# cg-tuwien/ppsurf

Hardware: AMD Instinct MI355X
Metric: occupancy query-points/sec @ res=257, 50NN (higher is better)
Workload: dtype f16x3

## Files before the change

include/ppsurf_amd_ext.h:

```cpp
#ifndef PPSURF_AMD_EXT_H
#define PPSURF_AMD_EXT_H
#include <stddef.h>
#include <stdint.h>

#ifdef __cplusplus
extern "C" {
#endif

int ppsx_blend_rgba_u8(const int64_t* idx, const float* d2, int64_t m, int k, const uint8_t* rgba, int64_t n, double eps, uint8_t* out,
                       void* stream);

int ppsx_trim_cell_slots(const float* pts, int64_t n, const float* lo, const float* hi, float h, float inv_h, uint64_t* table, int64_t capacity,
                         int64_t* slot, void* stream);
int ppsx_trim_face_support(const float* verts, int64_t nv, const int64_t* faces, int64_t nf, const float* pts, int64_t n, const float* lo,
                           const float* hi, float h, float inv_h, const uint64_t* table, int64_t capacity, const int64_t* order,
                           const int64_t* offsets, double r, uint8_t* support, void* stream);

int ppsx_smooth_half_edges(const int64_t* faces, int64_t nf, int64_t nv, int64_t* keys, void* stream);
int ppsx_smooth_pass(const double* x, int64_t nv, const int64_t* offsets, const int32_t* nbr, const int32_t* mult, int64_t ne, double s,
                     double* out, void* stream);

#ifdef __cplusplus
}
#endif
#endif
```

ppsurf_amd/build.py:

```python
import concurrent.futures
import os
import subprocess
import sys

HERE = os.path.dirname(os.path.abspath(__file__))
CSRC = os.path.join(HERE, 'csrc')
LIB = os.path.join(HERE, 'libppsurf_amd.so')
SOURCES = ['pps_decode.hip', 'pps_knn.hip', 'pps_grow.hip', 'pps_mc.hip', 'pps_mesh.hip', 'pps_fkaconv.hip', 'pps_sample.hip', 'pps_train.hip', 'pps_csr.hip', 'pps_fka_train.hip', 'pps_bn_train.hip',
           'pps_attn_train.hip', 'pps_rows_train.hip', 'pps_gemm_train.hip', 'pps_optim.hip', 'pps_eval.hip', 'pps_vis.hip', 'pps_scan.hip', 'pps_cloud.hip', 'pps_simplify.hip', 'pps_transfer.hip', 'pps_trim.hip', 'pps_smooth.hip', 'pps_pack.cpp']
HEADERS = ['pps_common.h', 'pps_fka_common.h', 'pps_rows_train_impl.h', 'pps_head_chain_impl.h', 'pps_sweep.h', 'pps_rng.h', 'pps_cells.h', 'pps_tri.h', os.path.join('..', '..', 'include', 'ppsurf_amd.h'),
           os.path.join('..', '..', 'include', 'ppsurf_amd_ext.h')]
FLAGS = ['--offload-arch=gfx950', '-O3', '-std=c++17', '-ffp-contract=off', '-fPIC']


def _newer(path, deps):
    if not os.path.isfile(path):
        return True
    t = os.path.getmtime(path)
    return any(os.path.getmtime(d) > t for d in deps if os.path.isfile(d))


def build(force=False, verbose=False, variant=None, defines=()):
    hipcc = os.environ.get('HIPCC', '/opt/rocm/bin/hipcc')
    lib = LIB if not variant else os.path.join(HERE, 'libppsurf_amd_{}.so'.format(variant))
    objdir = os.path.join(CSRC, 'build' + ('_' + variant if variant else ''))
    os.makedirs(objdir, exist_ok=True)
    headers = [os.path.join(CSRC, h) for h in HEADERS]
    srcs = [s for s in SOURCES if os.path.isfile(os.path.join(CSRC, s))]
    jobs = []
    for s in srcs:
        src, obj = os.path.join(CSRC, s), os.path.join(objdir, os.path.splitext(s)[0] + '.o')
        if force or _newer(obj, [src] + headers):
            jobs.append([hipcc] + FLAGS + list(defines) + ['-c', src, '-o', obj])
    if jobs:
        def run(cmd):
            if verbose:
                print(' '.join(cmd), flush=True)
            return subprocess.run(cmd, stdout=subprocess.PIPE, stderr=subprocess.STDOUT, text=True)
        with concurrent.futures.ThreadPoolExecutor(max_workers=min(8, len(jobs))) as pool:
            for res in pool.map(run, jobs):
                if res.returncode != 0:
                    sys.stderr.write(res.stdout)
                    raise subprocess.CalledProcessError(res.returncode, res.args)
                if verbose and res.stdout.strip():
                    print(res.stdout)
    objs = [os.path.join(objdir, os.path.splitext(s)[0] + '.o') for s in srcs]
    if jobs or _newer(lib, objs):
        subprocess.check_call([hipcc, '--offload-arch=gfx950', '-shared', '-fPIC'] + objs + ['-o', lib])
    return lib


if __name__ == '__main__':
    argv = sys.argv[1:]
    variant, defines = None, [a for a in argv if a.startswith(('-D', '-f', '-m'))]
    if '--variant' in argv:
        variant = argv[argv.index('--variant') + 1]
    print(build(force='--force' in argv, verbose=True, variant=variant, defines=defines))
```

ppsurf_amd/csrc/pps_decode.hip:

```cpp
#include <cstdlib>
#include "pps_common.h"
#include "../../include/ppsurf_amd.h"

using namespace pps;

#ifndef NT
#define NT 256
#endif
#define NW (NT / 64)
#ifndef WG_PER_CU
#define WG_PER_CU (512 / NT)
#endif
#ifndef PPS_PRIO
#define PPS_PRIO 1
#endif
#ifndef PPS_PRIO_PN
#define PPS_PRIO_PN 1
#endif
#define CH4 2048

template <int CHUNK_F4_NEXT, int NTH = NT, class F>
__device__ __forceinline__ void stream_step(const f32x4* __restrict__ gnext, f32x4*& cur, f32x4*& nxt, F&& compute) {
    chunk_copy_async<CHUNK_F4_NEXT / NTH, NTH>(gnext, nxt);
    compute((const f32x4*)cur);
    stream_wait();
    __syncthreads();
    f32x4* t = cur; cur = nxt; nxt = t;
}

template <int CHUNK_F4_NEXT, int NTH = NT, class F>
__device__ __forceinline__ void stream_step_spread(const f32x4* __restrict__ gnext, f32x4*& cur, f32x4*& nxt, F&& compute) {
    f32x4* dst = nxt;
    compute((const f32x4*)cur, [&](int i) { if (i < CHUNK_F4_NEXT / NTH) chunk_copy_piece<NTH>(gnext, dst, i); });
    stream_wait();
    __syncthreads();
    f32x4* t = cur; cur = nxt; nxt = t;
}

template <int CHUNK_F4_NEXT, int NTH = NT, class F>
__device__ __forceinline__ void stream_step_spread_at(const char* chunk, const unsigned (&voff)[CHUNK_F4_NEXT / NTH], f32x4*& cur, f32x4*& nxt, F&& compute) {
    f32x4* dst = nxt;
    compute((const f32x4*)cur, [&](int i) { if (i < CHUNK_F4_NEXT / NTH) chunk_copy_piece_at<NTH>(chunk, dst, i, voff[i]); });
    stream_wait();
    __syncthreads();
    f32x4* t = cur; cur = nxt; nxt = t;
}

template <int CHUNK_F4, int NTH = NT>
__device__ __forceinline__ void stream_prologue(const f32x4* __restrict__ g, f32x4* buf) {
    chunk_copy_async<CHUNK_F4 / NTH, NTH>(g, buf);
}

__device__ __forceinline__ void lds_fill(float* dst, const float* __restrict__ src, int nfloats) {
    for (int i = threadIdx.x; i < nfloats; i += blockDim.x) dst[i] = src[i];
}
// ... 1195 lines not shown
    if (q < 0) return PPS_ERR_ARG;
    if (q == 0) return PPS_OK;
    if (!g || !wpack || !bias || !trans2) return PPS_ERR_ARG;
    static int once = set_lds(pointnet_stn_fc_kernel, PB_LDS_BYTES);
    (void)once;
    hipLaunchKernelGGL(pointnet_stn_fc_kernel, dim3(grid_for((q + NW * 16 * PB_T - 1) / (NW * 16 * PB_T))), dim3(NT), PB_LDS_BYTES, (hipStream_t)stream,
                       g, q, wpack, bias, trans2, gate);
    return PPS_LAUNCH_CHECK();
}

static int decode_tail_f32_impl(const float* pooled, const float* xbar, int64_t q, const float* wpack, const float* bias,
                                float* logits, float* occ, int* gate, void* stream) {
    if (q < 0) return PPS_ERR_ARG;
    if (q == 0) return PPS_OK;
    if (!pooled || !xbar || !wpack || !bias || !logits) return PPS_ERR_ARG;
    static int once = set_lds(decode_tail_kernel, TL_LDS_BYTES);
    (void)once;
    hipLaunchKernelGGL(decode_tail_kernel, dim3(grid_for((q + NW * 16 - 1) / (NW * 16))), dim3(NT), TL_LDS_BYTES, (hipStream_t)stream,
                       pooled, xbar, q, wpack, bias, logits, occ, gate);
    return PPS_LAUNCH_CHECK();
}

extern "C" {

int pps_abi_version(void) { return 2; }

int pps_debug_occupancy(int which) {
    int n = -1;
    if (which == 0) { set_lds(interp_pool_kernel, IP_LDS_BYTES); hipOccupancyMaxActiveBlocksPerMultiprocessor(&n, interp_pool_kernel, NT, IP_LDS_BYTES); }
    if (which == 1) { set_lds(pointnet_stn_rows_kernel<false>, PA_LDS_BYTES); hipOccupancyMaxActiveBlocksPerMultiprocessor(&n, pointnet_stn_rows_kernel<false>, PNT, PA_LDS_BYTES); }
    if (which == 3) { set_lds(pointnet_stn_fc_kernel, PB_LDS_BYTES); hipOccupancyMaxActiveBlocksPerMultiprocessor(&n, pointnet_stn_fc_kernel, NT, PB_LDS_BYTES); }
    if (which == 4) { set_lds(pointnet_stn_fc_h_kernel, PB_LDS_BYTES); hipOccupancyMaxActiveBlocksPerMultiprocessor(&n, pointnet_stn_fc_h_kernel, NT, PB_LDS_BYTES); }
    if (which == 2) { set_lds(pointnet_feat_rows_kernel<false>, PC_LDS_BYTES); hipOccupancyMaxActiveBlocksPerMultiprocessor(&n, pointnet_feat_rows_kernel<false>, PNT, PC_LDS_BYTES); }
    return n;
}
int pps_device_cu_count(void) { return cu_count(); }

int pps_rows_dense256_f32(const float* in, int64_t rs, int64_t cs, int64_t m, const float* wpack, const float* bias,
                          float* out, void* stream) {
    if (m < 0) return PPS_ERR_ARG;
    if (m == 0) return PPS_OK;
    if (!in || !wpack || !bias || !out) return PPS_ERR_ARG;
    if (cs == 1 && (rs % 4) != 0) return PPS_ERR_ARG;
    static int once = set_lds(rows_dense256_kernel, RD_LDS_BYTES);
    (void)once;
    hipLaunchKernelGGL(rows_dense256_kernel, dim3(grid_for((m + NW * 16 - 1) / (NW * 16))), dim3(NT), RD_LDS_BYTES, (hipStream_t)stream,
                       in, rs, cs, m, wpack, bias, out);
    return PPS_LAUNCH_CHECK();
}

int pps_interp_pool_f32(const float* G, const float* pts, const float* query, const int64_t* idx, int64_t q, int k,
                        const float* wpack, const float* bias, float* pooled, void* stream) {
    return interp_pool_f32_impl(G, pts, query, idx, q, k, wpack, bias, pooled, nullptr, stream);
}

int pps_interp_pool_f16x3(const float* G, const float* pts, const float* query, const int64_t* idx, int64_t q, int k,
                          const float* wxyz, const void* w16, const float* bias, float* pooled, int32_t* range_flag, void* stream) {
    if (q < 0 || k < 1 || k > 64) return PPS_ERR_ARG;
    if (q == 0) return PPS_OK;
    if (!G || !pts || !query || !idx || !wxyz || !w16 || !bias || !pooled) return PPS_ERR_ARG;
    static int once = set_lds(interp_pool_f16x3_kernel, IH_LDS_BYTES);
    (void)once;
    int cus = cu_count();
    if (cus <= 0) cus = 256;
    const int64_t ntiles = (q + IH_NW / 4 - 1) / (IH_NW / 4);
    const int64_t wgs = (int64_t)cus * IH_WG_PER_CU;
    const int grid = (int)(ntiles < wgs ? ntiles : wgs);
    hipLaunchKernelGGL(interp_pool_f16x3_kernel, dim3(grid), dim3(IH_NT), IH_LDS_BYTES, (hipStream_t)stream,
                       G, pts, query, idx, q, k, wxyz, (const f32x4*)w16, bias, pooled, (int*)range_flag);
    return PPS_LAUNCH_CHECK();
}

int pps_interp_small_f32(const float* G, const float* pts, const float* query, const int64_t* idx, int64_t q, int k, int c,
                         const float* wpack, const float* bias, const float* wtail, int nout, float* out, void* stream) {
    if (q < 0 || k < 1 || k > 64 || (c != 32 && c != 64) || nout < 1 || nout > IS_MAX_OUT) return PPS_ERR_ARG;
    if (q == 0) return PPS_OK;
    if (!G || !pts || !query || !idx || !wpack || !bias || !wtail || !out) return PPS_ERR_ARG;
    int cus = cu_count();
    if (cus <= 0) cus = 256;
    const int grid = (int)(q < (int64_t)cus * 8 ? q : (int64_t)cus * 8);
    hipStream_t st = (hipStream_t)stream;
    if (c == 32) hipLaunchKernelGGL((interp_small_kernel<2, false>), dim3(grid), dim3(IS_NT), 0, st, G, pts, query, idx, q, k, wpack, nullptr, bias, wtail, nout, out, nullptr);
    else hipLaunchKernelGGL((interp_small_kernel<4, false>), dim3(grid), dim3(IS_NT), 0, st, G, pts, query, idx, q, k, wpack, nullptr, bias, wtail, nout, out, nullptr);
    return PPS_LAUNCH_CHECK();
}

int pps_interp_small_f16x3(const float* G, const float* pts, const float* query, const int64_t* idx, int64_t q, int k, int c,
                           const float* wpack, const void* w16, const float* bias, const float* wtail, int nout, float* out, int* guard,
                           void* stream) {
    if (q < 0 || k < 1 || k > 64 || (c != 32 && c != 64) || nout < 1 || nout > IS_MAX_OUT) return PPS_ERR_ARG;
    if (q == 0) return PPS_OK;
    if (!G || !pts || !query || !idx || !wpack || !w16 || !bias || !wtail || !out || !guard) return PPS_ERR_ARG;
    int cus = cu_count();
    if (cus <= 0) cus = 256;
    const int grid = (int)(q < (int64_t)cus * 8 ? q : (int64_t)cus * 8);
    hipStream_t st = (hipStream_t)stream;
    if (hipMemsetAsync(guard, 0, sizeof(int), st) != hipSuccess) return PPS_ERR_LAUNCH;
    const float* wh = (const float*)w16;
    if (c == 32) {
        hipLaunchKernelGGL((interp_small_kernel<2, true>), dim3(grid), dim3(IS_NT), 0, st, G, pts, query, idx, q, k, wpack, wh, bias, wtail, nout, out, guard);
        hipLaunchKernelGGL((interp_small_kernel<2, false>), dim3(grid), dim3(IS_NT), 0, st, G, pts, query, idx, q, k, wpack, nullptr, bias, wtail, nout, out, guard);
    } else {
        hipLaunchKernelGGL((interp_small_kernel<4, true>), dim3(grid), dim3(IS_NT), 0, st, G, pts, query, idx, q, k, wpack, wh, bias, wtail, nout, out, guard);
        hipLaunchKernelGGL((interp_small_kernel<4, false>), dim3(grid), dim3(IS_NT), 0, st, G, pts, query, idx, q, k, wpack, nullptr, bias, wtail, nout, out, guard);
    }
    return PPS_LAUNCH_CHECK();
// ... 145 lines not shown
```

ppsurf_amd/csrc/pps_knn.hip:

```cpp
#include "pps_common.h"
#include "../../include/ppsurf_amd.h"

#define KNN_QW 8
#define KNN_WAVES 4
#define KNN_CAP 128
#ifndef KNN_BISECT
#define KNN_BISECT 12
#endif
#ifndef KNN_SEED
#define KNN_SEED 4
#endif

typedef unsigned long long u64;

__device__ __forceinline__ u64 shfl_xor_u64(u64 v, int m) {
    const int lo = __shfl_xor((int)(unsigned)v, m), hi = __shfl_xor((int)(unsigned)(v >> 32), m);
    return ((u64)(unsigned)hi << 32) | (unsigned)lo;
}
__device__ __forceinline__ u64 shfl_u64(u64 v, int src) {
    const int lo = __shfl((int)(unsigned)v, src), hi = __shfl((int)(unsigned)(v >> 32), src);
    return ((u64)(unsigned)hi << 32) | (unsigned)lo;
}

__device__ __forceinline__ float wave_min_f32(float v, int lane) {
    v = fminf(v, pps::dpp_mov<0xB1>(v));
    v = fminf(v, pps::dpp_mov<0x4E>(v));
    v = fminf(v, pps::dpp_mov<0x141>(v));
    v = fminf(v, pps::dpp_mov<0x140>(v));
    v = fminf(v, __uint_as_float(pps::lane_xor_u32(__float_as_uint(v), 16, lane)));
    v = fminf(v, __uint_as_float(pps::lane_xor_u32(__float_as_uint(v), 32, lane)));
    return v;
}

__device__ __forceinline__ u64 wave_sort64(u64 key, int lane) {
#pragma unroll
    for (int size = 2; size <= 64; size <<= 1) {
#pragma unroll
        for (int st = size >> 1; st > 0; st >>= 1) {
            const u64 other = pps::lane_xor_u64(key, st, lane);
            const bool up = ((lane & size) == 0);
            const bool lower = ((lane & st) == 0);
            const bool take_min = (up == lower);
            const u64 mn = key < other ? key : other, mx = key < other ? other : key;
            key = take_min ? mn : mx;
        }
    }
    return key;
}
__device__ __forceinline__ u64 wave_bitonic_merge64(u64 key, int lane) {
#pragma unroll
    for (int st = 32; st > 0; st >>= 1) {
        const u64 other = pps::lane_xor_u64(key, st, lane);
        const bool lower = ((lane & st) == 0);
        const u64 mn = key < other ? key : other, mx = key < other ? other : key;
        key = lower ? mn : mx;
    }
    return key;
}

__device__ __forceinline__ u64 knn_flush(u64 list, const u64* cand, int cnt, int lane) {
    while (cnt > 0) {
        const int c = cnt < 64 ? cnt : 64;
        u64 ck = (lane < c) ? cand[cnt - c + lane] : ~0ull;
// ... 31 lines not shown
            const int p = base + lane;
            const bool pv = p < n;
            const int pc = pv ? p : n - 1;
            const float px = pts[3 * pc], py = pts[3 * pc + 1], pz = pts[3 * pc + 2];
#pragma unroll
            for (int j = 0; j < KNN_QW; ++j) {
                const float dx = __fsub_rn(qx[j], px), dy = __fsub_rn(qy[j], py), dz = __fsub_rn(qz[j], pz);
                const float d2 = __fadd_rn(__fadd_rn(__fmul_rn(dx, dx), __fmul_rn(dy, dy)), __fmul_rn(dz, dz));
                const bool pass = pv && (d2 < tau[j]);
                const u64 mask = __ballot(pass);
                if (mask != 0ull) {
                    u64* cand = cand_all[wave][j];
                    const int pos = cnt[j] + (int)__builtin_amdgcn_mbcnt_hi((unsigned)(mask >> 32), __builtin_amdgcn_mbcnt_lo((unsigned)mask, 0));
                    if (pass) cand[pos] = ((u64)__float_as_uint(d2) << 32) | (unsigned)p;
                    cnt[j] += __popcll(mask);
                    if (cnt[j] > KNN_CAP - 64) {
                        list[j] = knn_flush(list[j], cand + (cnt[j] - 64), 64, lane);
                        cnt[j] -= 64;
                        tau[j] = __uint_as_float((unsigned)(shfl_u64(list[j], k - 1) >> 32));
                    }
                }
            }
        }
#pragma unroll
        for (int j = 0; j < KNN_QW; ++j) {
            list[j] = knn_flush(list[j], cand_all[wave][j], cnt[j], lane);
            if (q0 + j < m && lane < k) {
                out_idx[(q0 + j) * k + lane] = (int64_t)(unsigned)(list[j] & 0xffffffffull);
                if (out_d2) out_d2[(q0 + j) * k + lane] = __uint_as_float((unsigned)(list[j] >> 32));
            }
        }
    }
}

__device__ __forceinline__ void wave_merge2(u64& a, u64& b, int lane) {
    const u64 rev = shfl_u64(b, 63 - lane);
    const u64 lo = a < rev ? a : rev, hi = a < rev ? rev : a;
    a = wave_bitonic_merge64(lo, lane);
    b = wave_bitonic_merge64(hi, lane);
}

template <int R>
__device__ __forceinline__ void knn_flush_r(u64 (&list)[R], const u64* cand, int cnt, int lane) {
    while (cnt > 0) {
        const int c = cnt < 64 ? cnt : 64;
        u64 carry = (lane < c) ? cand[cnt - c + lane] : ~0ull;
        carry = wave_sort64(carry, lane);
#pragma unroll
        for (int r = 0; r < R; ++r) wave_merge2(list[r], carry, lane);
        cnt -= c;
    }
}

template <int R>
__global__ __launch_bounds__(KNN_WAVES * 64) void knn_blocked_kernel(const float* __restrict__ pts, const int* __restrict__ orig,
                                                                     const float* __restrict__ bbox, int nb,
                                                                     const float* __restrict__ win_bbox, int n_win,
                                                                     const float* __restrict__ sbox ,
                                                                     const float* __restrict__ query, int64_t m, int k,
                                                                     int64_t* __restrict__ out_idx, float* __restrict__ out_d2) {
    __shared__ u64 cand_all[KNN_WAVES][KNN_QW][KNN_CAP];
    const int ngrp = (nb + 63) >> 6;
    const int lane = threadIdx.x & 63, wave = threadIdx.x >> 6;
    const int kr = (k - 1) >> 6, kl = (k - 1) & 63;
    const int64_t ntask = (m + KNN_QW - 1) / KNN_QW;
    for (int64_t task = (int64_t)blockIdx.x * KNN_WAVES + wave; task < ntask; task += (int64_t)gridDim.x * KNN_WAVES) {
        const int64_t q0 = task * KNN_QW;
        float qx[KNN_QW], qy[KNN_QW], qz[KNN_QW], tau[KNN_QW];
        u64 list[KNN_QW][R];
        int cnt[KNN_QW], wbest[KNN_QW];
#pragma unroll
        for (int j = 0; j < KNN_QW; ++j) {
            const int64_t qq = (q0 + j < m) ? q0 + j : m - 1;
            qx[j] = __shfl(query[qq * 3], 0); qy[j] = __shfl(query[qq * 3 + 1], 0); qz[j] = __shfl(query[qq * 3 + 2], 0);
            tau[j] = INFINITY;
            wbest[j] = 0;
#pragma unroll
            for (int r = 0; r < R; ++r) list[j][r] = ~0ull;
            cnt[j] = 0;
        }
        if (sbox != nullptr && n_win > 0) {
#pragma unroll
            for (int j = 0; j < KNN_QW; ++j) {
                float best = INFINITY;
                int bw = 0;
                for (int g0 = 0; g0 * 64 < n_win; g0 += 64) {
                    const int g = g0 + lane;
                    const bool gv = g * 64 < n_win;
                    const float* gb = sbox + (int64_t)(gv ? g : 0) * 6;
                    const float gx = fmaxf(fmaxf(__fsub_rn(gb[0], qx[j]), __fsub_rn(qx[j], gb[3])), 0.f);
                    const float gy = fmaxf(fmaxf(__fsub_rn(gb[1], qy[j]), __fsub_rn(qy[j], gb[4])), 0.f);
                    const float gz = fmaxf(fmaxf(__fsub_rn(gb[2], qz[j]), __fsub_rn(qz[j], gb[5])), 0.f);
                    const float gnear = gv ? __fadd_rn(__fadd_rn(__fmul_rn(gx, gx), __fmul_rn(gy, gy)), __fmul_rn(gz, gz)) : INFINITY;
                    u64 pend = __ballot(gnear < best);
                    while (pend != 0ull) {
                        const bool mine = (pend >> lane) & 1ull;
                        const float tn = wave_min_f32(mine ? gnear : INFINITY, lane);
                        const int src = __builtin_ctzll(__ballot(mine && gnear == tn));
                        const int b = (g0 + src) * 64 + lane;
                        const bool bv = b < n_win;
                        const float* bb = win_bbox + (int64_t)(bv ? b : 0) * 6;
                        const float fx = fmaxf(fabsf(__fsub_rn(qx[j], bb[0])), fabsf(__fsub_rn(qx[j], bb[3])));
                        const float fy = fmaxf(fabsf(__fsub_rn(qy[j], bb[1])), fabsf(__fsub_rn(qy[j], bb[4])));
                        const float fz = fmaxf(fabsf(__fsub_rn(qz[j], bb[2])), fabsf(__fsub_rn(qz[j], bb[5])));
                        const float far2 = bv ? __fadd_rn(__fadd_rn(__fmul_rn(fx, fx), __fmul_rn(fy, fy)), __fmul_rn(fz, fz)) : INFINITY;
                        const float tf = wave_min_f32(far2, lane);
                        if (tf < best) {
                            best = tf;
                            bw = (g0 + src) * 64 + __builtin_ctzll(__ballot(far2 == tf));
                        }
                        pend &= ~(1ull << src);
                        pend &= __ballot(gnear < best);
                    }
                }
                tau[j] = best;
                wbest[j] = bw;
            }
        } else {
            for (int b0 = 0; b0 < n_win; b0 += 64) {
                const int b = b0 + lane;
                const bool bv = b < n_win;
                const float* bb = win_bbox + (int64_t)(bv ? b : 0) * 6;
                const float lx = bb[0], ly = bb[1], lz = bb[2], hx = bb[3], hy = bb[4], hz = bb[5];
#pragma unroll
                for (int j = 0; j < KNN_QW; ++j) {
                    const float fx = fmaxf(fabsf(__fsub_rn(qx[j], lx)), fabsf(__fsub_rn(qx[j], hx)));
                    const float fy = fmaxf(fabsf(__fsub_rn(qy[j], ly)), fabsf(__fsub_rn(qy[j], hy)));
                    const float fz = fmaxf(fabsf(__fsub_rn(qz[j], lz)), fabsf(__fsub_rn(qz[j], hz)));
                    const float far2 = bv ? __fadd_rn(__fadd_rn(__fmul_rn(fx, fx), __fmul_rn(fy, fy)), __fmul_rn(fz, fz)) : INFINITY;
                    if (far2 < tau[j]) { tau[j] = far2; wbest[j] = b; }
                }
            }
        }
        const int nfull = n_win > 0 ? n_win + R - 1 : 0;
        constexpr int SEEDS = KNN_SEED > R ? KNN_SEED : R;
        const int nseed = nfull < SEEDS ? nfull : SEEDS;
#pragma unroll
        for (int j = 0; j < KNN_QW; ++j) {
            const float t = wave_min_f32(tau[j], lane);
            const u64 who = __ballot(tau[j] == t);
            tau[j] = t;
            if (nseed > 0) {
                const int w = __shfl(wbest[j], who != 0ull ? __builtin_ctzll(who) : 0);
                int s0 = w - (nseed - R) / 2;
                s0 = s0 < 0 ? 0 : s0;
                s0 = s0 + nseed > nfull ? nfull - nseed : s0;
                unsigned u[SEEDS];
#pragma unroll
                for (int rr = 0; rr < SEEDS; ++rr) {
                    const int p = (s0 + (rr < nseed ? rr : 0)) * 64 + lane;
                    const float dx = __fsub_rn(qx[j], pts[3 * p]), dy = __fsub_rn(qy[j], pts[3 * p + 1]), dz = __fsub_rn(qz[j], pts[3 * p + 2]);
                    const float d2 = __fadd_rn(__fadd_rn(__fmul_rn(dx, dx), __fmul_rn(dy, dy)), __fmul_rn(dz, dz));
                    u[rr] = rr < nseed ? __float_as_uint(d2) : 0xffffffffu;
                }
                unsigned lo = 0u, hi = __float_as_uint(tau[j]);
                {
                    int c = 0;
#pragma unroll
                    for (int rr = 0; rr < SEEDS; ++rr) c += __popcll(__ballot(u[rr] <= hi));
                    if (c < k) lo = hi;
                }
#pragma unroll
                for (int it = 0; it < KNN_BISECT; ++it) {
                    const unsigned mid = lo + ((hi - lo) >> 1);
                    int c = 0;
#pragma unroll
                    for (int rr = 0; rr < SEEDS; ++rr) c += __popcll(__ballot(u[rr] <= mid));
                    if (c >= k) hi = mid; else lo = mid + (lo < hi ? 1u : 0u);
                }
                tau[j] = __uint_as_float(hi);
            }
        }
        for (int g0 = 0; g0 < ngrp; g0 += 64) {
          u64 gneed[KNN_QW];
          u64 gany = 0ull;
          {
            const int g = g0 + lane;
            const bool gv = g < ngrp;
            if (sbox != nullptr) {
                const float* bb = sbox + (int64_t)(gv ? g : 0) * 6;
                const float lx = bb[0], ly = bb[1], lz = bb[2], hx = bb[3], hy = bb[4], hz = bb[5];
#pragma unroll
                for (int j = 0; j < KNN_QW; ++j) {
                    const float gx = fmaxf(fmaxf(__fsub_rn(lx, qx[j]), __fsub_rn(qx[j], hx)), 0.f);
                    const float gy = fmaxf(fmaxf(__fsub_rn(ly, qy[j]), __fsub_rn(qy[j], hy)), 0.f);
                    const float gz = fmaxf(fmaxf(__fsub_rn(lz, qz[j]), __fsub_rn(qz[j], hz)), 0.f);
                    const float near2 = __fadd_rn(__fadd_rn(__fmul_rn(gx, gx), __fmul_rn(gy, gy)), __fmul_rn(gz, gz));
                    gneed[j] = __ballot(gv && near2 <= tau[j]);
                    gany |= gneed[j];
                }
            } else {
                gany = __ballot(gv);
#pragma unroll
                for (int j = 0; j < KNN_QW; ++j) gneed[j] = gany;
            }
          }
          while (gany != 0ull) {
            const int gbit = __builtin_ctzll(gany);
            gany &= gany - 1ull;
            const int b0 = (g0 + gbit) * 64;
            const int b = b0 + lane;
            const bool bv = b < nb;
            const float* bb = bbox + (int64_t)(bv ? b : 0) * 6;
            const float lx = bb[0], ly = bb[1], lz = bb[2], hx = bb[3], hy = bb[4], hz = bb[5];
            u64 need[KNN_QW];
            u64 any = 0ull;
#pragma unroll
            for (int j = 0; j < KNN_QW; ++j) {
                need[j] = 0ull;
                if (((gneed[j] >> gbit) & 1ull) == 0ull) continue;
                const float gx = fmaxf(fmaxf(__fsub_rn(lx, qx[j]), __fsub_rn(qx[j], hx)), 0.f);
                const float gy = fmaxf(fmaxf(__fsub_rn(ly, qy[j]), __fsub_rn(qy[j], hy)), 0.f);
                const float gz = fmaxf(fmaxf(__fsub_rn(lz, qz[j]), __fsub_rn(qz[j], hz)), 0.f);
                const float near2 = __fadd_rn(__fadd_rn(__fmul_rn(gx, gx), __fmul_rn(gy, gy)), __fmul_rn(gz, gz));
                need[j] = __ballot(bv && near2 <= tau[j]);
                any |= need[j];
            }
            while (any != 0ull) {
                const int bit = __builtin_ctzll(any);
                any &= any - 1ull;
                const int p = (b0 + bit) * 64 + lane;
                const float px = pts[3 * p], py = pts[3 * p + 1], pz = pts[3 * p + 2];
                const int oi = orig[p];
                const bool pv = oi >= 0;
#pragma unroll
                for (int j = 0; j < KNN_QW; ++j) {
                    if (((need[j] >> bit) & 1ull) == 0ull) continue;
                    const float dx = __fsub_rn(qx[j], px), dy = __fsub_rn(qy[j], py), dz = __fsub_rn(qz[j], pz);
                    const float d2 = __fadd_rn(__fadd_rn(__fmul_rn(dx, dx), __fmul_rn(dy, dy)), __fmul_rn(dz, dz));
                    const bool pass = pv && (d2 <= tau[j]);
                    const u64 mask = __ballot(pass);
                    if (mask != 0ull) {
                        u64* cand = cand_all[wave][j];
                        const int pos = cnt[j] + (int)__builtin_amdgcn_mbcnt_hi((unsigned)(mask >> 32), __builtin_amdgcn_mbcnt_lo((unsigned)mask, 0));
                        if (pass) cand[pos] = ((u64)__float_as_uint(d2) << 32) | (unsigned)oi;
                        cnt[j] += __popcll(mask);
                        if (cnt[j] > KNN_CAP - 64) {
                            knn_flush_r<R>(list[j], cand + (cnt[j] - 64), 64, lane);
                            cnt[j] -= 64;
                            u64 kth = list[j][R - 1];
#pragma unroll
                            for (int r = 0; r + 1 < R; ++r) kth = (r == kr) ? list[j][r] : kth;
                            tau[j] = fminf(tau[j], __uint_as_float((unsigned)(shfl_u64(kth, kl) >> 32)));
                        }
                    }
                }
            }
          }
        }
#pragma unroll
        for (int j = 0; j < KNN_QW; ++j) {
            knn_flush_r<R>(list[j], cand_all[wave][j], cnt[j], lane);
            if (q0 + j < m) {
#pragma unroll
                for (int r = 0; r < R; ++r) {
                    const int e = r * 64 + lane;
                    if (e < k) {
                        out_idx[(q0 + j) * k + e] = (int64_t)(unsigned)(list[j][r] & 0xffffffffull);
                        if (out_d2) out_d2[(q0 + j) * k + e] = __uint_as_float((unsigned)(list[j][r] >> 32));
                    }
                }
            }
        }
    }
}

#define KBB_MAX 8
struct KbbKind {
    const float* pts; const int* orig; const float* bbox; const float* win; const float* query; const int* q_orig; int64_t* out;
    int64_t pts_stride, orig_stride, bbox_stride, win_stride, query_stride, qorig_stride, out_stride;
    int nb, n_win, m, k, groups, group_end;
};
struct KbbArgs { KbbKind kind[KBB_MAX]; int nkinds, nclouds; };

__global__ __launch_bounds__(KNN_WAVES * 64) void knn_blocked_batch_kernel(const KbbArgs a) {
    __shared__ u64 cand_all[KNN_WAVES][KNN_QW][KNN_CAP];
    const int lane = threadIdx.x & 63, wave = threadIdx.x >> 6;
    const int total = a.kind[a.nkinds - 1].group_end;
    for (int grp = blockIdx.x * KNN_WAVES + wave; grp < total; grp += gridDim.x * KNN_WAVES) {
        int t = 0;
        while (grp >= a.kind[t].group_end) ++t;
        const KbbKind& kd = a.kind[t];
        const int local = grp - (t == 0 ? 0 : a.kind[t - 1].group_end);
        const int cloud = local / kd.groups, q0 = (local % kd.groups) * KNN_QW;
        const float* __restrict__ pts = kd.pts + cloud * kd.pts_stride;
        const int* __restrict__ orig = kd.orig + cloud * kd.orig_stride;
        const float* __restrict__ bbox = kd.bbox + cloud * kd.bbox_stride;
        const float* __restrict__ win_bbox = kd.win + cloud * kd.win_stride;
        const float* __restrict__ query = kd.query + cloud * kd.query_stride;
        const int nb = kd.nb, n_win = kd.n_win, m = kd.m, k = kd.k;
        float qx[KNN_QW], qy[KNN_QW], qz[KNN_QW], tau[KNN_QW];
        u64 list[KNN_QW];
        int cnt[KNN_QW];
#pragma unroll
        for (int j = 0; j < KNN_QW; ++j) {
            const int qq = (q0 + j < m) ? q0 + j : m - 1;
// ... 198 lines not shown
```

ppsurf_amd/decoder.py:

```python
import ctypes

import numpy as np
import torch

from . import _lib

BN_EPS = 1e-5
C = 256
HEADS = 64


def _np64(t):
    if isinstance(t, torch.Tensor):
        t = t.detach().cpu().numpy()
    return np.asarray(t, dtype=np.float64)


def _fold_bn(w, b, sd, bn):
    scale = _np64(sd[bn + '.weight']) / np.sqrt(_np64(sd[bn + '.running_var']) + BN_EPS)
    return w * scale[:, None], (b - _np64(sd[bn + '.running_mean'])) * scale + _np64(sd[bn + '.bias'])


def _wb(sd, name):
    w = _np64(sd[name + '.weight'])
# ... 128 lines not shown
                t[:16].copy_(old[:16])
            self._scratch[name] = t
        return t[:n].view(shape)

    def intermediates(self, q):
        ws = self.scratch('decode_ws', (_lib.lib().pps_decode_ws_bytes(q) // 4,))
        sizes = (('pooled', C), ('g', C), ('trans2', 4096), ('xbar', C))
        out, off = {}, 16
        for name, width in sizes:
            out[name] = ws[off:off + q * width].view(q, width) if name != 'xbar' else ws[off:off + q * 128].view(q, 128)
            off += q * width
        return out

    def point_table(self, latents_cn):
        latents = latents_cn
        assert latents.dim() == 2 and latents.shape[0] == C and latents.dtype == torch.float32 and latents.device == self.device
        n, rs, cs = latents.shape[1], latents.stride(1), latents.stride(0)
        if cs == 1 and rs % 4 != 0:
            raise ValueError('point-major latents need a row stride that is a multiple of 4 floats')
        out = torch.empty((n, C), dtype=torch.float32, device=self.device)
        _lib.call('pps_rows_dense256_f32', latents, rs, cs, n, self.w['g_w'], self.w['g_b'], out)
        return out

    def decode(self, table, pts, query, idx, patches, want_occ=True, stage_events=None, lane=0):
        L = _lib.lib()
        q, k, p = query.shape[0], idx.shape[1], patches.shape[1]
        for t in (table, pts, query, idx, patches):
            assert t.is_contiguous() and t.device == self.device
        logits = torch.empty((q, 2), dtype=torch.float32, device=self.device)
        occ = torch.empty((q,), dtype=torch.float32, device=self.device) if want_occ else None
        ws = self.scratch('decode_ws' if lane == 0 else 'decode_ws{}'.format(lane), (L.pps_decode_ws_bytes(q) // 4,))
        if getattr(self, '_wptrs', None) is None:
            self._wptrs = (ctypes.c_void_p * 10)(*[self.w[n].data_ptr() for n in ('ip_w', 'ip_b', 'pa_w', 'pa_b', 'pb_w', 'pb_b', 'pc_w',
                                                                                  'pc_b', 'tl_w', 'tl_b')])
        args = (table, pts, query, idx, q, k, patches, p, self._wptrs, logits, occ, ws)
        if self.w16 is not None:
            _lib.call('pps_decode_fwd_mixed_f32', *args[:9], self.w16, *args[9:], stage_events)
        elif stage_events is None:
            _lib.call('pps_decode_fwd_f32', *args)
        else:
            _lib.call('pps_decode_fwd_events_f32', *args, stage_events)
        return logits, occ

    def range_fallbacks(self):
        if self.w16 is None:
            return 0
        return sum(int(ws[:16].view(torch.int32)[1]) for name, ws in self._scratch.items() if name.startswith('decode_ws'))


class ChunkPipeline:

    LANE_MIN_CHUNKS = 4

    def __init__(self, plan: DecoderPlan, table, pts, raw, k: int, p: int, same_cloud: bool, max_chunk: int, overlap: bool = False, lanes=None):
        from . import ops
        import os
        self.ops, self.plan, self.table, self.pts, self.raw = ops, plan, table, pts, raw
        self.k, self.p, self.same_cloud, self.overlap = int(k), int(p), bool(same_cloud), bool(overlap)
        env = os.environ.get('PPS_CHUNK_LANES')
        self.lanes = int(env) if env else lanes
        self.max_chunk = int(max_chunk)
        self.idx, self.patches = [], []
        self.pidx = None if (same_cloud and self.p <= self.k) else []
        self._grow_buffers(2)
        self.blocks = self.ops.KnnBlocks(pts)
        self.raw_blocks = None if self.pidx is None else self.ops.KnnBlocks(raw)
        dev = plan.device
        self.side = torch.cuda.Stream(device=dev) if overlap else None
        self.lane_streams = []
        self.ready = [torch.cuda.Event() for _ in range(2)]
        self.free = [torch.cuda.Event() for _ in range(2)]
        self.n = 0

    def _grow_buffers(self, count):
        dev = self.plan.device
        while len(self.idx) < count:
            self.idx.append(torch.empty((self.max_chunk, self.k), dtype=torch.int64, device=dev))
            self.patches.append(torch.empty((self.max_chunk, self.p, 3), dtype=torch.float32, device=dev))
            if self.pidx is not None:
                self.pidx.append(torch.empty((self.max_chunk, self.p), dtype=torch.int64, device=dev))

    def _spatial(self, q, b):
        m = q.shape[0]
        idx = self.idx[b][:m]
        if self.pidx is not None and self.same_cloud and self.p > self.k:
            src = self.pidx[b][:m]
            self.raw_blocks.query(q, self.p, out=src)
            idx.copy_(src[:, :self.k])
        else:
            self.blocks.query(q, self.k, out=idx)
            src = idx
            if self.pidx is not None:
                src = self.pidx[b][:m]
                self.raw_blocks.query(q, self.p, out=src)
        self.ops.patch_normalize(self.raw, q, src, self.p, out=self.patches[b][:m])

    def _run_lanes(self, chunks, want_occ, lanes):
        dev = self.plan.device
        main = torch.cuda.current_stream(dev)
        while len(self.lane_streams) < lanes:
            self.lane_streams.append(torch.cuda.Stream(device=dev))
        self._grow_buffers(max(lanes, 2))
        out = [None] * len(chunks)
        for ln in range(lanes):
            st = self.lane_streams[ln]
            st.wait_stream(main)
            with torch.cuda.stream(st):
                for i in range(ln, len(chunks), lanes):
                    q = chunks[i]
                    m = q.shape[0]
                    self._spatial(q, ln)
                    out[i] = self.plan.decode(self.table, self.pts, q, self.idx[ln][:m], self.patches[ln][:m], want_occ=want_occ, lane=ln)
        for ln in range(lanes):
            main.wait_stream(self.lane_streams[ln])
        for lg, oc in out:
            lg.record_stream(main)
            if oc is not None:
                oc.record_stream(main)
        return out

    def run(self, chunks, want_occ=True, stage_events=None):
        lanes = self.lanes if self.lanes is not None else (2 if len(chunks) >= self.LANE_MIN_CHUNKS else 1)
        if stage_events is None and lanes > 1 and len(chunks) > 1 and self.side is None:
            res = self._run_lanes(chunks, want_occ, min(lanes, len(chunks)))
            self.n += len(chunks)
            return res
        main = torch.cuda.current_stream(self.plan.device)
        out = []
        for i, q in enumerate(chunks):
            b = (self.n + i) & 1
            if self.side is not None:
                self.side.wait_stream(main) if i == 0 else None
                with torch.cuda.stream(self.side):
                    self.side.wait_event(self.free[b])
                    self._spatial(q, b)
                    self.ready[b].record(self.side)
                main.wait_event(self.ready[b])
            else:
                self._spatial(q, b)
            m = q.shape[0]
            ev = stage_events[i] if stage_events is not None else None
            out.append(self.plan.decode(self.table, self.pts, q, self.idx[b][:m], self.patches[b][:m], want_occ=want_occ, stage_events=ev))
            self.free[b].record(main)
        self.n += len(chunks)
        return out


class PocoDecoderPlan:

    DTYPES = ('f32', 'f16x3')

    def __init__(self, sd, device, prefix='projection', dtype=None):
        import os
        self.dtype = dtype or os.environ.get('PPS_DECODER_DTYPE', 'f16x3')
        if self.dtype not in self.DTYPES:
            raise ValueError('decoder dtype must be one of {} (got {!r})'.format(self.DTYPES, self.dtype))
        p = prefix
        w1, b1 = _wb(sd, p + '.fc1')
        c = w1.shape[0]
        if c not in (32, 64) or w1.shape[1] != c + 3:
            raise NotImplementedError('the small-latent HIP decoder handles latent sizes 32 and 64 (got fc1 {})'.format(w1.shape))
        w2, b2 = _wb(sd, p + '.fc2')
        w3, b3 = _wb(sd, p + '.fc3')
        wq, bq = _wb(sd, p + '.fc_query')
        wv, bv = _wb(sd, p + '.fc_value')
        w8, b8 = _wb(sd, p + '.fc8')
        if wq.shape[0] != HEADS or w8.shape[0] > 8:
# ... 38 lines not shown
```

Measured before the change: 12.56 million.

## Prefetch kNN spatial queries on side streams and slim kNN ballot masks

Each decode lane gets a dedicated spatial stream that runs kNN and patch normalisation for upcoming chunks. Double-buffered index and patch buffers, synchronised with ready and free events, let the next chunk's neighbour search overlap with the current decode. Separately, the R==1 kNN kernel keeps per-lane query bitmasks and uses readfirstlane/readlane instead of one 64-bit ballot per query. This cuts register pressure and ballot work. The build also gains kernel resource-usage reporting, and a small LDS-size query function is added.

Measured after the change: 12.50 million. Within noise of the previous version (-0.5%).

```diff
diff --git a/include/ppsurf_amd_ext.h b/include/ppsurf_amd_ext.h
--- a/include/ppsurf_amd_ext.h
+++ b/include/ppsurf_amd_ext.h
@@ -20,6 +20,8 @@
 int ppsx_smooth_pass(const double* x, int64_t nv, const int64_t* offsets, const int32_t* nbr, const int32_t* mult, int64_t ne, double s,
                      double* out, void* stream);
 
+int ppsx_interp_f16x3_lds_bytes(int* bytes);
+
 #ifdef __cplusplus
 }
 #endif
diff --git a/ppsurf_amd/build.py b/ppsurf_amd/build.py
--- a/ppsurf_amd/build.py
+++ b/ppsurf_amd/build.py
@@ -1,5 +1,7 @@
 import concurrent.futures
+import json
 import os
+import re
 import subprocess
 import sys
 
@@ -11,6 +13,11 @@
 HEADERS = ['pps_common.h', 'pps_fka_common.h', 'pps_rows_train_impl.h', 'pps_head_chain_impl.h', 'pps_sweep.h', 'pps_rng.h', 'pps_cells.h', 'pps_tri.h', os.path.join('..', '..', 'include', 'ppsurf_amd.h'),
            os.path.join('..', '..', 'include', 'ppsurf_amd_ext.h')]
 FLAGS = ['--offload-arch=gfx950', '-O3', '-std=c++17', '-ffp-contract=off', '-fPIC']
+RESOURCES = os.path.join(HERE, 'kernel_resources.json')
+RESOURCE_SOURCES = ('pps_knn.hip', 'pps_decode.hip')
+RESOURCE_FLAG = '-Rpass-analysis=kernel-resource-usage'
+_RESOURCE_KEYS = {'TotalSGPRs': 'sgprs', 'VGPRs': 'vgprs', 'AGPRs': 'agprs', 'ScratchSize [bytes/lane]': 'scratch_bytes_per_lane',
+                  'Occupancy [waves/SIMD]': 'waves_per_simd', 'LDS Size [bytes/block]': 'lds_bytes'}
 
 
 def _newer(path, deps):
@@ -18,6 +25,38 @@
         return True
     t = os.path.getmtime(path)
     return any(os.path.getmtime(d) > t for d in deps if os.path.isfile(d))
+
+
+def kernel_name(mangled):
+    m = re.match(r'_Z(\d+)', mangled)
+    if not m or m.end() + int(m.group(1)) > len(mangled):
+        return mangled
+    name, rest = mangled[m.end():m.end() + int(m.group(1))], mangled[m.end() + int(m.group(1)):]
+    if not rest.startswith('I'):
+        return name
+    args, rest = [], rest[1:]
+    while not rest.startswith('E'):
+        a = re.match(r'L([a-z])(n?)(\d+)E', rest)
+        if not a:
+            return mangled
+        val = ('-' if a.group(2) else '') + a.group(3)
+        args.append({'0': 'false', '1': 'true'}.get(val, val) if a.group(1) == 'b' else val)
+        rest = rest[a.end():]
+    return '{}<{}>'.format(name, ', '.join(args))
+
+
+def parse_resource_remarks(text):
+    out, cur = {}, None
+    for line in text.splitlines():
+        m = re.search(r'remark:\s+(.*?):\s+(\S+)\s+\[-Rpass-analysis=kernel-resource-usage\]', line)
+        if not m:
+            continue
+        key, val = m.group(1).strip(), m.group(2)
+        if key == 'Function Name':
+            cur = out.setdefault(kernel_name(val), {'symbol': val})
+        elif cur is not None and key in _RESOURCE_KEYS:
+            cur[_RESOURCE_KEYS[key]] = int(val)
+    return out
 
 
 def build(force=False, verbose=False, variant=None, defines=()):
@@ -30,23 +69,42 @@
     jobs = []
     for s in srcs:
         src, obj = os.path.join(CSRC, s), os.path.join(objdir, os.path.splitext(s)[0] + '.o')
-        if force or _newer(obj, [src] + headers):
-            jobs.append([hipcc] + FLAGS + list(defines) + ['-c', src, '-o', obj])
+        res = obj[:-2] + '.resources.json' if s in RESOURCE_SOURCES else None
+        if force or _newer(obj, [src] + headers) or (res and _newer(res, [obj])):
+            jobs.append(([hipcc] + FLAGS + ([RESOURCE_FLAG] if res else []) + list(defines) + ['-c', src, '-o', obj], res))
     if jobs:
-        def run(cmd):
+        def run(job):
             if verbose:
-                print(' '.join(cmd), flush=True)
-            return subprocess.run(cmd, stdout=subprocess.PIPE, stderr=subprocess.STDOUT, text=True)
+                print(' '.join(job[0]), flush=True)
+            return subprocess.run(job[0], stdout=subprocess.PIPE, stderr=subprocess.STDOUT, text=True)
         with concurrent.futures.ThreadPoolExecutor(max_workers=min(8, len(jobs))) as pool:
-            for res in pool.map(run, jobs):
+            for (cmd, respath), res in zip(jobs, pool.map(run, jobs)):
                 if res.returncode != 0:
                     sys.stderr.write(res.stdout)
                     raise subprocess.CalledProcessError(res.returncode, res.args)
-                if verbose and res.stdout.strip():
-                    print(res.stdout)
+                text = res.stdout
+                if respath:
+                    found = parse_resource_remarks(text)
+                    if not found:
+                        raise RuntimeError('{}: the compiler reported no kernel resources ({})'.format(cmd[-3], RESOURCE_FLAG))
+                    with open(respath, 'w') as f:
+                        json.dump(found, f, indent=1, sort_keys=True)
+                    text = '\n'.join(ln for ln in text.splitlines() if RESOURCE_FLAG not in ln)
+                if verbose and text.strip():
+                    print(text)
     objs = [os.path.join(objdir, os.path.splitext(s)[0] + '.o') for s in srcs]
     if jobs or _newer(lib, objs):
         subprocess.check_call([hipcc, '--offload-arch=gfx950', '-shared', '-fPIC'] + objs + ['-o', lib])
+    parts = [os.path.join(objdir, os.path.splitext(s)[0] + '.resources.json') for s in srcs if s in RESOURCE_SOURCES]
+    table = RESOURCES if not variant else os.path.join(HERE, 'kernel_resources_{}.json'.format(variant))
+    if _newer(table, parts):
+        kernels = {}
+        for part in parts:
+            with open(part) as f:
+                for name, v in json.load(f).items():
+                    kernels[name] = dict(v, source=os.path.basename(part)[:-len('.resources.json')] + '.hip')
+        with open(table, 'w') as f:
+            json.dump({'arch': 'gfx950', 'flags': FLAGS + list(defines), 'kernels': kernels}, f, indent=1, sort_keys=True)
     return lib
 
 
diff --git a/ppsurf_amd/csrc/pps_decode.hip b/ppsurf_amd/csrc/pps_decode.hip
--- a/ppsurf_amd/csrc/pps_decode.hip
+++ b/ppsurf_amd/csrc/pps_decode.hip
@@ -1,6 +1,7 @@
 #include <cstdlib>
 #include "pps_common.h"
 #include "../../include/ppsurf_amd.h"
+#include "../../include/ppsurf_amd_ext.h"
 
 using namespace pps;
 
@@ -1302,6 +1303,12 @@
 int pps_interp_pool_f32(const float* G, const float* pts, const float* query, const int64_t* idx, int64_t q, int k,
                         const float* wpack, const float* bias, float* pooled, void* stream) {
     return interp_pool_f32_impl(G, pts, query, idx, q, k, wpack, bias, pooled, nullptr, stream);
+}
+
+int ppsx_interp_f16x3_lds_bytes(int* bytes) {
+    if (!bytes) return PPS_ERR_ARG;
+    *bytes = (int)IH_LDS_BYTES;
+    return PPS_OK;
 }
 
 int pps_interp_pool_f16x3(const float* G, const float* pts, const float* query, const int64_t* idx, int64_t q, int k,
diff --git a/ppsurf_amd/csrc/pps_knn.hip b/ppsurf_amd/csrc/pps_knn.hip
--- a/ppsurf_amd/csrc/pps_knn.hip
+++ b/ppsurf_amd/csrc/pps_knn.hip
@@ -9,6 +9,9 @@
 #endif
 #ifndef KNN_SEED
 #define KNN_SEED 4
+#endif
+#ifndef KNN_SLIM
+#define KNN_SLIM 1
 #endif
 
 typedef unsigned long long u64;
@@ -146,6 +149,8 @@
     }
 }
 
+__device__ __forceinline__ float knn_uniform(float v) { return __uint_as_float(__builtin_amdgcn_readfirstlane(__float_as_uint(v))); }
+
 template <int R>
 __global__ __launch_bounds__(KNN_WAVES * 64) void knn_blocked_kernel(const float* __restrict__ pts, const int* __restrict__ orig,
                                                                      const float* __restrict__ bbox, int nb,
@@ -154,6 +159,7 @@
                                                                      const float* __restrict__ query, int64_t m, int k,
                                                                      int64_t* __restrict__ out_idx, float* __restrict__ out_d2) {
     __shared__ u64 cand_all[KNN_WAVES][KNN_QW][KNN_CAP];
+    constexpr bool SLIM = KNN_SLIM && (R == 1);
     const int ngrp = (nb + 63) >> 6;
     const int lane = threadIdx.x & 63, wave = threadIdx.x >> 6;
     const int kr = (k - 1) >> 6, kl = (k - 1) & 63;
@@ -166,7 +172,11 @@
 #pragma unroll
         for (int j = 0; j < KNN_QW; ++j) {
             const int64_t qq = (q0 + j < m) ? q0 + j : m - 1;
-            qx[j] = __shfl(query[qq * 3], 0); qy[j] = __shfl(query[qq * 3 + 1], 0); qz[j] = __shfl(query[qq * 3 + 2], 0);
+            if constexpr (SLIM) {
+                qx[j] = knn_uniform(query[qq * 3]); qy[j] = knn_uniform(query[qq * 3 + 1]); qz[j] = knn_uniform(query[qq * 3 + 2]);
+            } else {
+                qx[j] = __shfl(query[qq * 3], 0); qy[j] = __shfl(query[qq * 3 + 1], 0); qz[j] = __shfl(query[qq * 3 + 2], 0);
+            }
             tau[j] = INFINITY;
             wbest[j] = 0;
 #pragma unroll
@@ -233,7 +243,7 @@
         for (int j = 0; j < KNN_QW; ++j) {
             const float t = wave_min_f32(tau[j], lane);
             const u64 who = __ballot(tau[j] == t);
-            tau[j] = t;
+            tau[j] = SLIM ? knn_uniform(t) : t;
             if (nseed > 0) {
                 const int w = __shfl(wbest[j], who != 0ull ? __builtin_ctzll(who) : 0);
                 int s0 = w - (nseed - R) / 2;
@@ -266,7 +276,8 @@
             }
         }
         for (int g0 = 0; g0 < ngrp; g0 += 64) {
-          u64 gneed[KNN_QW];
+          u64 gneed[SLIM ? 1 : KNN_QW];
+          unsigned gq = 0u;
           u64 gany = 0ull;
           {
             const int g = g0 + lane;
@@ -280,46 +291,71 @@
                     const float gy = fmaxf(fmaxf(__fsub_rn(ly, qy[j]), __fsub_rn(qy[j], hy)), 0.f);
                     const float gz = fmaxf(fmaxf(__fsub_rn(lz, qz[j]), __fsub_rn(qz[j], hz)), 0.f);
                     const float near2 = __fadd_rn(__fadd_rn(__fmul_rn(gx, gx), __fmul_rn(gy, gy)), __fmul_rn(gz, gz));
-                    gneed[j] = __ballot(gv && near2 <= tau[j]);
-                    gany |= gneed[j];
-                }
+                    if constexpr (SLIM) {
+                        gq |= (gv && near2 <= tau[j]) ? (1u << j) : 0u;
+                    } else {
+                        gneed[j] = __ballot(gv && near2 <= tau[j]);
+                        gany |= gneed[j];
+                    }
+                }
+                if constexpr (SLIM) gany = __ballot(gq != 0u);
             } else {
                 gany = __ballot(gv);
-#pragma unroll
-                for (int j = 0; j < KNN_QW; ++j) gneed[j] = gany;
+                if constexpr (SLIM) {
+                    gq = gv ? (1u << KNN_QW) - 1u : 0u;
+                } else {
+#pragma unroll
+                    for (int j = 0; j < KNN_QW; ++j) gneed[j] = gany;
+                }
             }
           }
           while (gany != 0ull) {
             const int gbit = __builtin_ctzll(gany);
             gany &= gany - 1ull;
+            const unsigned gqm = SLIM ? __builtin_amdgcn_readlane(gq, gbit) : 0u;
             const int b0 = (g0 + gbit) * 64;
             const int b = b0 + lane;
             const bool bv = b < nb;
             const float* bb = bbox + (int64_t)(bv ? b : 0) * 6;
             const float lx = bb[0], ly = bb[1], lz = bb[2], hx = bb[3], hy = bb[4], hz = bb[5];
-            u64 need[KNN_QW];
+            u64 need[SLIM ? 1 : KNN_QW];
+            unsigned nq = 0u;
             u64 any = 0ull;
 #pragma unroll
             for (int j = 0; j < KNN_QW; ++j) {
-                need[j] = 0ull;
-                if (((gneed[j] >> gbit) & 1ull) == 0ull) continue;
+                if constexpr (SLIM) {
+                    if (((gqm >> j) & 1u) == 0u) continue;
+                } else {
+                    need[j] = 0ull;
+                    if (((gneed[j] >> gbit) & 1ull) == 0ull) continue;
+                }
                 const float gx = fmaxf(fmaxf(__fsub_rn(lx, qx[j]), __fsub_rn(qx[j], hx)), 0.f);
                 const float gy = fmaxf(fmaxf(__fsub_rn(ly, qy[j]), __fsub_rn(qy[j], hy)), 0.f);
                 const float gz = fmaxf(fmaxf(__fsub_rn(lz, qz[j]), __fsub_rn(qz[j], hz)), 0.f);
                 const float near2 = __fadd_rn(__fadd_rn(__fmul_rn(gx, gx), __fmul_rn(gy, gy)), __fmul_rn(gz, gz));
-                need[j] = __ballot(bv && near2 <= tau[j]);
-                any |= need[j];
-            }
+                if constexpr (SLIM) {
+                    nq |= (bv && near2 <= tau[j]) ? (1u << j) : 0u;
+                } else {
+                    need[j] = __ballot(bv && near2 <= tau[j]);
+                    any |= need[j];
+                }
+            }
+            if constexpr (SLIM) any = __ballot(nq != 0u);
             while (any != 0ull) {
                 const int bit = __builtin_ctzll(any);
                 any &= any - 1ull;
+                const unsigned nqm = SLIM ? __builtin_amdgcn_readlane(nq, bit) : 0u;
                 const int p = (b0 + bit) * 64 + lane;
                 const float px = pts[3 * p], py = pts[3 * p + 1], pz = pts[3 * p + 2];
                 const int oi = orig[p];
                 const bool pv = oi >= 0;
 #pragma unroll
                 for (int j = 0; j < KNN_QW; ++j) {
-                    if (((need[j] >> bit) & 1ull) == 0ull) continue;
+                    if constexpr (SLIM) {
+                        if (((nqm >> j) & 1u) == 0u) continue;
+                    } else {
+                        if (((need[j] >> bit) & 1ull) == 0ull) continue;
+                    }
                     const float dx = __fsub_rn(qx[j], px), dy = __fsub_rn(qy[j], py), dz = __fsub_rn(qz[j], pz);
                     const float d2 = __fadd_rn(__fadd_rn(__fmul_rn(dx, dx), __fmul_rn(dy, dy)), __fmul_rn(dz, dz));
                     const bool pass = pv && (d2 <= tau[j]);
@@ -335,7 +371,8 @@
                             u64 kth = list[j][R - 1];
 #pragma unroll
                             for (int r = 0; r + 1 < R; ++r) kth = (r == kr) ? list[j][r] : kth;
-                            tau[j] = fminf(tau[j], __uint_as_float((unsigned)(shfl_u64(kth, kl) >> 32)));
+                            const float tk = fminf(tau[j], __uint_as_float((unsigned)(shfl_u64(kth, kl) >> 32)));
+                            tau[j] = SLIM ? knn_uniform(tk) : tk;
                         }
                     }
                 }
diff --git a/ppsurf_amd/decoder.py b/ppsurf_amd/decoder.py
--- a/ppsurf_amd/decoder.py
+++ b/ppsurf_amd/decoder.py
@@ -204,13 +204,16 @@
 
     LANE_MIN_CHUNKS = 4
 
-    def __init__(self, plan: DecoderPlan, table, pts, raw, k: int, p: int, same_cloud: bool, max_chunk: int, overlap: bool = False, lanes=None):
+    def __init__(self, plan: DecoderPlan, table, pts, raw, k: int, p: int, same_cloud: bool, max_chunk: int, overlap: bool = False, lanes=None,
+                 spatial_ahead: bool = True):
         from . import ops
         import os
         self.ops, self.plan, self.table, self.pts, self.raw = ops, plan, table, pts, raw
         self.k, self.p, self.same_cloud, self.overlap = int(k), int(p), bool(same_cloud), bool(overlap)
         env = os.environ.get('PPS_CHUNK_LANES')
         self.lanes = int(env) if env else lanes
+        env = os.environ.get('PPS_SPATIAL_AHEAD')
+        self.spatial_ahead = bool(int(env)) if env else bool(spatial_ahead)
         self.max_chunk = int(max_chunk)
         self.idx, self.patches = [], []
         self.pidx = None if (same_cloud and self.p <= self.k) else []
@@ -219,7 +222,7 @@
         self.raw_blocks = None if self.pidx is None else self.ops.KnnBlocks(raw)
         dev = plan.device
         self.side = torch.cuda.Stream(device=dev) if overlap else None
-        self.lane_streams = []
+        self.lane_streams, self.spatial_streams = [], []
         self.ready = [torch.cuda.Event() for _ in range(2)]
         self.free = [torch.cuda.Event() for _ in range(2)]
         self.n = 0
@@ -252,11 +255,35 @@
         main = torch.cuda.current_stream(dev)
         while len(self.lane_streams) < lanes:
             self.lane_streams.append(torch.cuda.Stream(device=dev))
-        self._grow_buffers(max(lanes, 2))
+        ahead = self.spatial_ahead
+        if ahead:
+            while len(self.spatial_streams) < lanes:
+                self.spatial_streams.append(torch.cuda.Stream(device=dev))
+            while len(self.ready) < 2 * lanes:
+                self.ready.append(torch.cuda.Event())
+                self.free.append(torch.cuda.Event())
+        self._grow_buffers(2 * lanes if ahead else max(lanes, 2))
         out = [None] * len(chunks)
         for ln in range(lanes):
             st = self.lane_streams[ln]
             st.wait_stream(main)
+            if ahead:
+                sp = self.spatial_streams[ln]
+                sp.wait_stream(main)
+                for j, i in enumerate(range(ln, len(chunks), lanes)):
+                    q = chunks[i]
+                    m = q.shape[0]
+                    b = 2 * ln + (j & 1)
+                    with torch.cuda.stream(sp):
+                        if j >= 2:
+                            sp.wait_event(self.free[b])
+                        self._spatial(q, b)
+                        self.ready[b].record(sp)
+                    with torch.cuda.stream(st):
+                        st.wait_event(self.ready[b])
+                        out[i] = self.plan.decode(self.table, self.pts, q, self.idx[b][:m], self.patches[b][:m], want_occ=want_occ, lane=ln)
+                        self.free[b].record(st)
+                continue
             with torch.cuda.stream(st):
                 for i in range(ln, len(chunks), lanes):
                     q = chunks[i]
@@ -265,6 +292,8 @@
                     out[i] = self.plan.decode(self.table, self.pts, q, self.idx[ln][:m], self.patches[ln][:m], want_occ=want_occ, lane=ln)
         for ln in range(lanes):
             main.wait_stream(self.lane_streams[ln])
+            if ahead:
+                main.wait_stream(self.spatial_streams[ln])
         for lg, oc in out:
             lg.record_stream(main)
             if oc is not None:
```
